# Yuki-11/CSBSR

Hardware: AMD Instinct MI355X
Metric: training imgs/s (448->1792 x4, PSPNet) (higher is better)
Workload: dtype fp16 storage / fp32 accumulate (detector forward: split fp16 hi+lo); 1 GPU; CSBSR KBPN x4 + PSPNet, beta=0.3, joint phase (iter 40000), per-GPU batch 8, LR 448x448 -> HR 1792x1792, fwd+loss+bwd+Adam; batch resident in HBM (H2D outside `value`, timed beside it as with_h2d_inside_step); full-size synthetic crack images degraded on the device; global_batch=8, micro_batch=8, parallelism=dp1

## Files before the change

csbsr_amd/csrc/conv_common.h:

```cpp
#pragma once
#include "common.h"

struct ConvK {
  csbsr_seg_t in[2];
  int N, H, W, OH, OW;
  int transposed, KHt, KWt;
  int stride, pad, dil;
  int ctot, c0;
  int Kp;
  int rows_p;
  const half_t* wt;
  int cout, coutp;
  half_t* out16; long o_sn, o_sy, o_sx;
  float* out32; long o32_sn, o32_sy, o32_sx, o32_sc;
  const float* bias;
  const float* cbias;
  int cb_mode;
  int act; float act_slope; const float* prelu;
  int res_mode; const half_t* res; long r_sn, r_sy, r_sx;
  const half_t* res2; long r2_sn, r2_sy, r2_sx;
  int accumulate;
  int stat_mode; float* stat;
  float out_scale;
  unsigned tiles_m, tiles_n;
// ... 284 lines not shown
      }
    }
    return;
  }
  if constexpr (BNSTAT) return;
  constexpr int NBATCH = 4 * (4 / NB);
  h8 rr[2][NB], oo[2][NB], mm[2][NB];
  auto load_batch = [&](int b, int st) __attribute__((always_inline)) {
    const int mp = b / (4 / NB), nb = (b % (4 / NB)) * NB;
    const int co = co0 + 16 * mp;
    const int coc = co < p.coutp ? co : p.coutp - 8;
#pragma unroll
    for (int r = 0; r < NB; ++r) {
      const int oyr = oyc[nb + r];
      rr[st][r] = h8{0, 0, 0, 0, 0, 0, 0, 0}; oo[st][r] = h8{0, 0, 0, 0, 0, 0, 0, 0}; mm[st][r] = h8{1, 1, 1, 1, 1, 1, 1, 1};
      if (fe.has_res) rr[st][r] = *reinterpret_cast<const h8*>(p.res + n * p.r_sn + oyr * p.r_sy + oxc * p.r_sx + coc);
      if (fe.has_old) oo[st][r] = *reinterpret_cast<const h8*>(p.out16 + n * p.o_sn + oyr * p.o_sy + oxc * p.o_sx + coc);
      if (fe.has_mask) mm[st][r] = *reinterpret_cast<const h8*>(p.mask + n * p.m_sn + oyr * p.m_sy + oxc * p.m_sx + coc);
    }
  };
  load_batch(0, 0);
#pragma unroll
  for (int b = 0; b < NBATCH; ++b) {
    if (b + 1 < NBATCH) load_batch(b + 1, (b + 1) & 1);
    const int mp = b / (4 / NB), nb = (b % (4 / NB)) * NB;
    const int co = co0 + 16 * mp;
    const int coc = co < p.coutp ? co : p.coutp - 8;
#pragma unroll
    for (int r = 0; r < NB; ++r) {
      float v[8], t[8];
#pragma unroll
      for (int e = 0; e < 8; ++e) v[e] = acc[mp >> 1][nb + r][8 * (mp & 1) + e];
      conv_epilogue_fast_values<true, BNSTAT>(fe, v, bias[mp], co, rr[b & 1][r], oo[b & 1][r], bsum[mp], bsq[mp], mm[b & 1][r], t, valid[nb + r] && co < p.coutp);
      split_store_rs(rs, (rowoff[nb + r] + pixoff + 2 * coc) | (co >= p.coutp ? (int)0x80000000 : 0), fe.o_lo, t);
        __builtin_amdgcn_sched_barrier(0);
    }
  }
}
#endif

template <int CPR, int NW>
__device__ __forceinline__ void conv_epilogue_flush_stats(const ConvK& p, float* sStat, int BN, int local_col, int co, float (&ssum)[8], float (&ssq)[8]) {
  if (p.stat_mode == CSBSR_STAT_NONE) return;
  const bool sq = p.stat_mode == CSBSR_STAT_BN;
#pragma unroll
  for (int e = 0; e < 8; ++e) {
    float a = co < p.coutp ? ssum[e] : 0.f, b = (sq && co < p.coutp) ? ssq[e] : 0.f;
#pragma unroll
    for (int o = CPR; o < 64; o <<= 1) { a += __shfl_xor(a, o, 64); if (sq) b += __shfl_xor(b, o, 64); }
    ssum[e] = a; ssq[e] = b;
  }
  const int wid = threadIdx.x >> 6;
  const bool mine = (threadIdx.x & 63) < CPR && co < p.coutp;
#pragma unroll 1
  for (int w = 0; w < NW; ++w) {
    if (wid == w && mine) {
#pragma unroll
      for (int e = 0; e < 8; ++e) {
        sStat[local_col + e] += ssum[e];
        if (sq) sStat[BN + local_col + e] += ssq[e];
      }
    }
    lds_barrier();
  }
}
__device__ __forceinline__ void conv_epilogue_store_stats(const ConvK& p, const float* sStat, int BN, int cout0, size_t row) {
  const int tid = threadIdx.x;
  if (p.stat_mode == CSBSR_STAT_NONE || tid >= BN || cout0 + tid >= p.coutp) return;
  float* r = p.stat_part + row * p.stat_ld + cout0 + tid;
  r[0] = sStat[tid];
  if (p.stat_mode == CSBSR_STAT_BN) r[p.coutp] = sStat[BN + tid];
}
struct ConvStatPlan { long rows; int tps; };
static inline int conv_stat_prepare(ConvK& p, int BM, int nphase, ConvStatPlan& pl, hipStream_t st) {
  pl.rows = 0; pl.tps = 0;
  p.stat_part = nullptr; p.stat_ld = 0; p.hw_pad = 0;
  if (p.stat_mode == CSBSR_STAT_NONE) return 0;
  if (p.stat_mode == CSBSR_STAT_SAMPLE_SUM) {
    CSBSR_CHECK(!p.transposed, "conv: per-sample sums of a transposed convolution are not built");
    if (p.tile2d) pl.tps = (p.OW / 16) * (p.OH / (BM / 16));
    else {
      p.hw_pad = round_up(p.OH * p.OW, BM);
      pl.tps = p.hw_pad / BM;
      p.tiles_m = (unsigned)(p.N * pl.tps);
    }
  }
  pl.rows = (long)p.tiles_m * nphase;
  p.stat_ld = (p.stat_mode == CSBSR_STAT_BN ? 2 : 1) * (long)p.coutp;
  p.stat_part = csbsr_red_scratch(pl.rows * p.stat_ld);
  CSBSR_NEED_SCRATCH(p.stat_part, "conv (fused statistics)");
  if (p.transposed && hipMemsetAsync(p.stat_part, 0, (size_t)pl.rows * p.stat_ld * 4, st) != hipSuccess) {
    csbsr_set_error("conv: memset of the statistics rows failed");
    return 2;
  }
  return 0;
}
static inline int conv_stat_finish(const ConvK& p, const ConvStatPlan& pl, hipStream_t st) {
  if (p.stat_mode == CSBSR_STAT_BN) return csbsr_sum_partials(p.stat_part, (int)pl.rows, p.stat_ld, 2 * p.coutp, p.stat, st);
  if (p.stat_mode == CSBSR_STAT_SAMPLE_SUM) return csbsr_sum_partials_batched(p.stat_part, pl.tps, p.stat_ld, p.coutp, p.stat, p.N, p.coutp, st);
  return 0;
}

__device__ __forceinline__ void conv_epilogue_direct_tile(const ConvK& p, const f16v& acc, int cbase ,
                                                          float slope, int n, int oy, int ox, const float* bias_tab = nullptr,
                                                          const EpiFast* fe = nullptr) {
  if (n < 0) return;
  const int hi = (threadIdx.x & 63) >> 5;
#pragma unroll
  for (int pair = 0; pair < 2; ++pair) {
    float v[8];
#pragma unroll
    for (int j = 0; j < 4; ++j) {
      const unsigned a = __float_as_uint(acc[8 * pair + j]), b = __float_as_uint(acc[8 * pair + 4 + j]);
      auto r = __builtin_amdgcn_permlane32_swap(a, b, false, false);
      v[j] = __uint_as_float(r[0]);
      v[4 + j] = __uint_as_float(r[1]);
    }
    const int co = cbase + 16 * pair + 8 * hi;
    if (co >= p.coutp) continue;
    float bias[8];
#pragma unroll
    for (int e = 0; e < 8; ++e) bias[e] = bias_tab ? bias_tab[co + e] : ((p.bias && co + e < p.cout) ? p.bias[co + e] : 0.f);
    float s0[8], s1[8];
    if (fe && fe->ok && !fe->bn) {
      half_t* o = p.out16 + n * p.o_sn + oy * p.o_sy + ox * p.o_sx + co;
      h8 rr = {0, 0, 0, 0, 0, 0, 0, 0}, oo = {0, 0, 0, 0, 0, 0, 0, 0};
      if (fe->has_res) rr = *reinterpret_cast<const h8*>(p.res + n * p.r_sn + oy * p.r_sy + ox * p.r_sx + co);
      if (fe->has_old) oo = *reinterpret_cast<const h8*>(o);
      float brow[8];
      if (fe->has_cb) conv_class_bias_row(p, bias, co, n, oy, ox, brow);
      else {
#pragma unroll
        for (int e = 0; e < 8; ++e) brow[e] = bias[e];
      }
      if (fe->has_res || fe->has_old) conv_epilogue_fast_row<true, false>(*fe, v, brow, co, o, rr, oo, s0, s1);
      else conv_epilogue_fast_row<false, false>(*fe, v, brow, co, o, rr, oo, s0, s1);
      continue;
    }
    conv_epilogue_row(p, v, bias, slope, co, n, oy, ox, s0, s1);
  }
}

enum { CONVK_IGEMM32 = 0, CONVK_IGEMM64, CONVK_IGEMM128, CONVK_GLDS128, CONVK_GLDS256, CONVK_THIN_COUT, CONVK_THIN_CIN, CONVK_GLDS256W, CONVK_HR, CONVK_TP, CONVK_X3, CONVK_THIN_TP, CONVK_X3S, CONVK_THIN_CIN2, CONVK_GLDS64, CONVK_THIN_SC, CONVK_THIN_TPD, CONVK_X3F, CONVK_X3SF, CONVK_X3W, CONVK_X3N };
extern thread_local int g_last_conv_kernel;
int conv_desc_to_k(const csbsr_conv_desc_t* d, ConvK& k);
bool conv_thin_eligible(const ConvK& k);
int conv_thin_launch(const ConvK& k, hipStream_t st);
void conv_thin_enable(int on);
bool conv_thin_cin_eligible(const ConvK& k, int creal);
int conv_thin_cin_launch(const ConvK& k, int creal, hipStream_t st);
bool conv_thin_cin2_eligible(const ConvK& k, int creal);
int conv_thin_cin2_launch(const ConvK& k, int creal, hipStream_t st);
void conv_thin_cin2_enable(int on);
int conv_thin_cin2_dact_launch(const ConvK& k, const csbsr_conv_desc_t* d, hipStream_t st);
extern "C" int32_t csbsr_conv_thin_dact_eligible(const csbsr_conv_desc_t* d);
bool conv_thin_tp_eligible(const ConvK& k, int creal, bool second_seg);
int conv_thin_tp_launch(const ConvK& k, hipStream_t st);
bool conv_thin_sc_eligible(const ConvK& k);
int conv_thin_sc_launch(const ConvK& k, hipStream_t st);
void conv_thin_sc_enable(int on);
bool conv_thin_tpd_eligible(const ConvK& k, int KH);
int conv_thin_tpd_launch(const ConvK& k, int KH, hipStream_t st);
void conv_thin_tpd_enable(int on);
bool conv_glds_eligible(const ConvK& k);
int conv_glds_launch(const ConvK& k, int nphase, long maxM, hipStream_t st);
```

csbsr_amd/csrc/conv_igemm_glds.hip:

```cpp
#include "common.h"
#include "csbsr_debug.h"
#include "conv_common.h"
#include <type_traits>

#ifdef CSBSR_TS
__device__ unsigned long long g_ts[8 * 262144];
#define TS(i) do { if (threadIdx.x == 0 && blockIdx.x < 262144) g_ts[(size_t)blockIdx.x * 8 + (i)] = wall_clock64(); } while (0)
extern "C" int csbsr_debug_read_ts(void* dst, long n) { return (int)hipMemcpyFromSymbol(dst, HIP_SYMBOL(g_ts), n * 8); }
#else
#define TS(i)
#endif
template <int BM, int NWM, int NSTAGE, int CT = 1, bool FS = false, bool GK = false>
__global__ __launch_bounds__(NWM * 128) void conv_igemm_glds_kernel(const ConvK p, const half_t* __restrict__ zero_page) {
  constexpr int BN = CT ? 128 * CT : 64, BKG = 64;
  constexpr int TA = CT ? 2 * CT : 1;
  constexpr int SOW = BN > 128 ? 128 : BN;
  constexpr int NW = NWM * 2, NT = NW * 64;
  constexpr int XI = BM / 8, WI = BN / 8;
  constexpr int NI = (XI + WI) / NW;
  constexpr int NXI = XI / NW;
  constexpr int STAGE_BYTES = (BM + BN) * 128;
  constexpr int RING_BYTES = NSTAGE * STAGE_BYTES;
  constexpr int OUT_LD = 64 + 4;
  constexpr int EPI_BYTES = BM * SOW * 4;
// ... 330 lines not shown
#pragma unroll
  for (int a = 0; a < (TA < 2 ? TA : 2); ++a)
#pragma unroll
    for (int b = 0; b < 2; ++b) {
      const int pix = wm * 64 + b * 32 + (lane & 31);
#pragma unroll
      for (int q = 0; q < 4; ++q) {
        const int slot = (wn * (SOW / 2) + a * 32 + 8 * q + 4 * (lane >> 5)) >> 2;
        const f16v& t = acc[2 * hh + a][b];
        f4 v = {t[4 * q + 0], t[4 * q + 1], t[4 * q + 2], t[4 * q + 3]};
        *reinterpret_cast<f4*>(sO + pix * SOW + ((slot ^ (pix & 15)) << 2)) = v;
      }
    }
  lds_barrier();
  if (hh == 0) TS(5);
  const int lcol = CT != 2 ? cc8 * 8 : (cc8 >> 3) * 128 + hh * 64 + (cc8 & 7) * 8;
  const int co = cout0 + lcol;
  float bias[8], ssum[8], ssq[8];
#pragma unroll
  for (int e = 0; e < 8; ++e) { bias[e] = sBias[lcol + e]; ssum[e] = ssq[e] = 0.f; }
  if (fe.ok) {
    constexpr int RPT = BM / RSTEP, EG = CT == 2 ? 2 : (RPT < 8 ? RPT : 8);
    static_assert(RPT % EG == 0, "rows per thread must split into groups");
    auto rows = [&](auto EXTRA, auto BNSTAT) {
#pragma unroll 1
      for (int g = 0; g < RPT / EG; ++g) {
        h8 rr[EG], oo[EG], mm[EG];
        long ooff[EG];
        bool live[EG];
#pragma unroll
        for (int i = 0; i < EG; ++i) {
          const int grow = tid / CPR + (g * EG + i) * RSTEP;
          const int n = sRow[grow * 3];
          live[i] = n >= 0 && co < p.coutp;
          ooff[i] = sOOff[grow] + co;
          rr[i] = h8{0, 0, 0, 0, 0, 0, 0, 0}; oo[i] = h8{0, 0, 0, 0, 0, 0, 0, 0}; mm[i] = h8{1, 1, 1, 1, 1, 1, 1, 1};
          if constexpr (decltype(EXTRA)::value) {
            if (live[i]) {
              if (fe.has_res || fe.has_mask) {
                const int oyo = py + sRow[grow * 3 + 1] * o_step, oxo = px + sRow[grow * 3 + 2] * o_step;
                if (fe.has_res) rr[i] = *reinterpret_cast<const h8*>(p.res + n * p.r_sn + oyo * p.r_sy + oxo * p.r_sx + co);
                if (fe.has_mask) mm[i] = *reinterpret_cast<const h8*>(p.mask + n * p.m_sn + oyo * p.m_sy + oxo * p.m_sx + co);
              }
              if (fe.has_old) oo[i] = *reinterpret_cast<const h8*>(p.out16 + ooff[i]);
            }
          }
        }
#pragma unroll
        for (int i = 0; i < EG; ++i) {
          if (!live[i]) continue;
          const int row = tid / CPR + (g * EG + i) * RSTEP;
          const f4 v0 = *reinterpret_cast<const f4*>(sO + row * SOW + (((2 * cc8) ^ (row & 15)) << 2));
          const f4 v1 = *reinterpret_cast<const f4*>(sO + row * SOW + (((2 * cc8 + 1) ^ (row & 15)) << 2));
          const float v[8] = {v0[0], v0[1], v0[2], v0[3], v1[0], v1[1], v1[2], v1[3]};
          if (fe.has_cb) {
            float brow[8];
            conv_class_bias_row(p, bias, co, sRow[row * 3], py + sRow[row * 3 + 1] * o_step, px + sRow[row * 3 + 2] * o_step, brow);
            conv_epilogue_fast_row<decltype(EXTRA)::value, decltype(BNSTAT)::value>(fe, v, brow, co, p.out16 + ooff[i], rr[i], oo[i], ssum, ssq, mm[i]);
            continue;
          }
          conv_epilogue_fast_row<decltype(EXTRA)::value, decltype(BNSTAT)::value>(fe, v, bias, co, p.out16 + ooff[i], rr[i], oo[i], ssum, ssq, mm[i]);
        }
      }
    };
    const bool extra = fe.has_res || fe.has_old || fe.has_mask;
    if (fe.bn) { if (extra) rows(std::true_type{}, std::true_type{}); else rows(std::false_type{}, std::true_type{}); }
    else { if (extra) rows(std::true_type{}, std::false_type{}); else rows(std::false_type{}, std::false_type{}); }
    if (fe.bn) conv_epilogue_flush_stats<CPR, NW>(p, sStat, BN, lcol, co, ssum, ssq);
  } else {
    constexpr int RPT = BM / RSTEP, EG = 2;
#pragma unroll 1
    for (int g = 0; g < RPT / EG; ++g) {
      EpiPre pre[EG];
      int rn[EG], roy[EG], rox[EG];
#pragma unroll
      for (int i = 0; i < EG; ++i) {
        const int grow = tid / CPR + (g * EG + i) * RSTEP;
        const int n = sRow[grow * 3];
        rn[i] = (n < 0 || co >= p.coutp) ? -1 : n;
        roy[i] = py + sRow[grow * 3 + 1] * o_step;
        rox[i] = px + sRow[grow * 3 + 2] * o_step;
        if (rn[i] >= 0) conv_epilogue_prefetch(p, co, rn[i], roy[i], rox[i], pre[i]);
      }
#pragma unroll
      for (int i = 0; i < EG; ++i) {
        if (rn[i] < 0) continue;
        const int row = tid / CPR + (g * EG + i) * RSTEP;
        float v[8];
        const f4 v0 = *reinterpret_cast<const f4*>(sO + row * SOW + (((2 * cc8) ^ (row & 15)) << 2));
        const f4 v1 = *reinterpret_cast<const f4*>(sO + row * SOW + (((2 * cc8 + 1) ^ (row & 15)) << 2));
        v[0] = v0[0]; v[1] = v0[1]; v[2] = v0[2]; v[3] = v0[3]; v[4] = v1[0]; v[5] = v1[1]; v[6] = v1[2]; v[7] = v1[3];
        conv_epilogue_row(p, v, bias, slope, co, rn[i], roy[i], rox[i], ssum, ssq, &pre[i]);
      }
    }
    conv_epilogue_flush_stats<CPR, NW>(p, sStat, BN, lcol, co, ssum, ssq);
  }
  };
  epi_pass(std::integral_constant<int, 0>{});
  if constexpr (CT == 2) epi_pass(std::integral_constant<int, 1>{});
  TS(6);
  conv_epilogue_store_stats(p, sStat, BN, cout0, (size_t)zph * p.tiles_m + tile_m);
}

static half_t* g_zero_page = nullptr;
static int g_glds_phase_flat = 1;
static int g_glds_tile2d = 1;
static int g_glds_tap_group = 1;
static int g_glds_wide = 1;
static int g_glds_narrow = 1;
static int g_glds_gk = 1;

template <int BM, int NWM, int NSTAGE, int CT = 1, bool FS = false, bool GK = false>
static int launch_glds(const ConvK& k, int nphase, long maxM, hipStream_t st) {
  ConvK p = k;
  constexpr int BN = CT ? 128 * CT : 64, SOW = BN > 128 ? 128 : BN;
  p.tiles_m = (unsigned)((maxM + BM - 1) / BM);
  p.tile2d = (g_glds_tile2d && !k.transposed && k.KHt * k.KWt > 1 && k.OW % 16 == 0 && k.OH % (BM / 16) == 0) ? 1 : 0;
  p.tap_group = (!GK && g_glds_tap_group && !k.transposed && k.stride > 1 && k.dil == 1 && k.KHt > k.stride && k.KHt % k.stride == 0 &&
                 k.KWt > k.stride && k.KWt % k.stride == 0) ? 1 : 0;
  p.tiles_n = (unsigned)((k.coutp + BN - 1) / BN);
  constexpr int RING = NSTAGE * (BM + BN) * 128;
  constexpr int EPI = BM * SOW * 4;
  constexpr int SM_BYTES = (RING > EPI ? RING : EPI) + BM * (4 * 8 + 3 * 4) + 3 * BN * 4 + (GK ? 64 * 8 : 0);
  static_assert(SM_BYTES <= 160 * 1024, "LDS budget");
  static LdsAttrOnce attr;
  if (int e = csbsr_lds_attr(attr, reinterpret_cast<const void*>(conv_igemm_glds_kernel<BM, NWM, NSTAGE, CT, FS, GK>), SM_BYTES, "conv(glds)")) return e;
  if (!g_zero_page) {
    if (hipMalloc(reinterpret_cast<void**>(&g_zero_page), 256) != hipSuccess) { csbsr_set_error("conv(glds): zero page alloc failed"); return 2; }
    (void)hipMemset(g_zero_page, 0, 256);
  }
  p.nphase_flat = (g_glds_phase_flat && nphase > 1) ? nphase : 0;
  ConvStatPlan sp;
  if (int e = conv_stat_prepare(p, BM, nphase, sp, st)) return e;
  dim3 grid(p.tiles_m * p.tiles_n * (p.nphase_flat ? nphase : 1), 1, p.nphase_flat ? 1 : nphase);
  hipLaunchKernelGGL((conv_igemm_glds_kernel<BM, NWM, NSTAGE, CT, FS, GK>), grid, dim3(NWM * 128), SM_BYTES, st, p, g_zero_page);
  if (int e = conv_stat_finish(p, sp, st)) return e;
  CSBSR_LAUNCH_CHECK("csbsr_conv_forward(glds)");
  return 0;
}

static int g_glds_mode = 2;
extern "C" void csbsr_debug_set_conv_glds(int mode) {
  g_glds_mode = mode & 7;
  g_glds_phase_flat = (mode & 32) ? 0 : 1;
  g_glds_tap_group = (mode & 128) ? 0 : 1;
  g_glds_tile2d = (mode & 64) ? 0 : 1;
  g_glds_wide = (mode & 256) ? 0 : 1;
  g_glds_narrow = (mode & 1024) ? 0 : 1;
  g_glds_gk = (mode & 2048) ? 0 : 1;
  conv_thin_enable((mode & 16) ? 0 : 1);
  conv_thin_sc_enable((mode & 4096) ? 0 : 1);
  conv_thin_tpd_enable((mode & 8192) ? 0 : 1);
  conv_thin_cin2_enable((mode & 512) ? 0 : 1);
}

static bool conv_glds_general_k(const ConvK& k) { return k.fs ? (k.ctot / 2) % 32 != 0 : k.ctot % 64 != 0; }

bool conv_glds_eligible(const ConvK& k) {
  if (g_glds_mode == 0) return false;
  if (k.coutp <= 32 || (k.coutp <= 64 && !g_glds_narrow)) return false;
  if (conv_glds_general_k(k)) {
    if (!g_glds_gk || k.c0 != k.ctot || (k.fs ? k.ctot / 2 : k.ctot) < 32) return false;
  } else if (k.c0 != k.ctot && k.c0 % 64 != 0) return false;
  if (k.rows_p % (k.coutp <= 64 ? 64 : 128) != 0) return false;
  if (k.KHt * k.KWt > 64) return false;
  return true;
}

int conv_glds_launch(const ConvK& k, int nphase, long maxM, hipStream_t st) {
  const bool big = (g_glds_mode == 2 && !k.transposed && k.Kp >= 2304 && maxM >= 256 * 256) ||
                   (g_glds_mode == 2 && !k.transposed && k.Kp >= 512 && k.coutp >= 384 && maxM >= (1l << 22)) ||
                   (g_glds_mode == 3 && maxM >= 256 * 256);
  const int pad128 = (k.coutp + 127) / 128 * 128, pad256 = (k.coutp + 255) / 256 * 256;
  const bool wide = big && g_glds_wide && k.coutp >= 256 && pad256 * 8 <= pad128 * 9 + 64;
  const bool gk = conv_glds_general_k(k);
  const int tile = k.coutp <= 64 ? 0 : (!big ? 1 : (wide ? 3 : 2));
  g_last_conv_kernel = (tile == 0 ? CONVK_GLDS64 : (tile == 1 ? CONVK_GLDS128 : (tile == 3 ? CONVK_GLDS256W : CONVK_GLDS256))) |
                       ((k.fs ? 1 : 0) | (gk ? 2 : 0)) << 8;
#define GLDS_DISPATCH(FS_, GK_)                                                                      \
  switch (tile) {                                                                                    \
    case 0: return launch_glds<128, 2, 2, 0, FS_, GK_>(k, nphase, maxM, st);                        \
    case 1: return launch_glds<128, 2, 2, 1, FS_, GK_>(k, nphase, maxM, st);                        \
    case 3: return launch_glds<256, 4, 2, 2, FS_, GK_>(k, nphase, maxM, st);                        \
    default: return launch_glds<256, 4, 3, 1, FS_, GK_>(k, nphase, maxM, st);                       \
  }
  if (k.fs) { if (gk) { GLDS_DISPATCH(true, true) } else { GLDS_DISPATCH(true, false) } }
  if (gk) { GLDS_DISPATCH(false, true) }
  GLDS_DISPATCH(false, false)
#undef GLDS_DISPATCH
}
```

csbsr_amd/csrc/conv_thin.hip:

```cpp
#include "conv_common.h"

#define TN_TH 8
#define TN_TW 32
#define TN_HW (TN_TW + 2)
#define TN_HP ((TN_TH + 2) * TN_HW)
#define TN_MB ((TN_HP + 31) / 32)
#define TN_YLD 33

#define TN_TPW 1

__global__ __launch_bounds__(256) void conv_thin_cout_kernel(const ConvK p, int tiles_x, int tiles_y, int wld) {
  extern __shared__ __attribute__((aligned(16))) char smem[];
  half_t* sW = reinterpret_cast<half_t*>(smem);
  float* sY = reinterpret_cast<float*>(smem + (size_t)32 * wld * sizeof(half_t));
  const int tid = threadIdx.x, lane = tid & 63, wid = tid >> 6;
  int b = blockIdx.x;
  const int tx = b % tiles_x; b /= tiles_x;
  const int tyg = (tiles_y + TN_TPW - 1) / TN_TPW;
  const int ty0 = (b % tyg) * TN_TPW;
  const int n = b / tyg;
  const int CR = p.cout, ntap_rows = 9 * CR;

  {
    const int chunks_per_row = wld / 8;
// ... 250 lines not shown
  }
  const float aslope = p.act == CSBSR_ACT_RELU ? 0.f : (p.act == CSBSR_ACT_LRELU ? p.act_slope : 1.f);
  const float mslope = DACT ? *x.slope : 1.f, rsign = p.res_mode == CSBSR_RES_SUB ? -1.f : 1.f;
  float dpr = 0.f;
  const half_t* in0 = reinterpret_cast<const half_t*>(p.in[0].ptr);
  const unsigned per_img = (unsigned)(tiles_x * tiles_y), total = per_img * (unsigned)p.N;
  auto halo_load = [&](unsigned t) {
    h8 v = {0, 0, 0, 0, 0, 0, 0, 0};
    if (tid < TN_HP && t < total) {
      const int n = t / per_img;
      const unsigned r = t - n * per_img;
      const int hy = tid / TN_HW, hx = tid - hy * TN_HW;
      const int iy = (int)(r / tiles_x) * TN_TH + hy - 1, ix = (int)(r % tiles_x) * TN_TW + hx - 1;
      if ((unsigned)iy < (unsigned)p.H && (unsigned)ix < (unsigned)p.W)
        v = *reinterpret_cast<const h8*>(in0 + (long)n * p.in[0].sn + (long)iy * p.in[0].sy + (long)ix * p.in[0].sx);
    }
    return v;
  };
  unsigned t = blockIdx.x;
  if (t >= total) return;
  {
    const h8 v = halo_load(t);
    if (tid < TN_HP) *reinterpret_cast<h8*>(sIn + tid * 8) = v;
  }
  __syncthreads();
  int buf = 0;
  for (; t < total; t += gridDim.x) {
    const h8 hnext = halo_load(t + gridDim.x);
    const int n = t / per_img;
    const unsigned r_ = t - n * per_img;
    const int oy = (int)(r_ / tiles_x) * TN_TH + wid, ox = (int)(r_ % tiles_x) * TN_TW + pix;
    const bool live = oy < p.OH && ox < p.OW;
    const half_t* sI = sIn + buf * (TN_HP * 8);
    h8 pf[2];
#pragma unroll
    for (int s = 0; s < 2; ++s)
#pragma unroll
      for (int e = 0; e < 8; ++e) {
        const int k = 16 * s + 8 * hi + e;
        const int tap = k / CI, c = k - tap * CI;
        const int ky = tap / 3, kx = tap - ky * 3;
        pf[s][e] = tap < 9 ? sI[((wid + ky) * TN_HW + pix + kx) * 8 + c] : (half_t)0;
      }
    half_t* o = p.out16 + (live ? n * p.o_sn + oy * p.o_sy + ox * p.o_sx : 0) + 8 * hi;
    h8 ring[RD][2];
    h8 ringm[DACT ? RD : 1][2], ringr[DACT ? RD : 1][2];
    const half_t* mo = DACT ? p.mask + (live ? n * p.m_sn + oy * p.m_sy + ox * p.m_sx : 0) + 8 * hi : nullptr;
    const half_t* ro = DACT ? p.res + (live ? n * p.r_sn + oy * p.r_sy + ox * p.r_sx : 0) + 8 * hi : nullptr;
    half_t* dro = DACT ? x.dres + (live ? n * x.d_sn + oy * x.d_sy + ox * x.d_sx : 0) + 8 * hi : nullptr;
    auto piece_ok = [&](int ct, int pair) { return 32 * ct + 16 * pair + 8 * hi < p.coutp; };
    if (has_old) {
#pragma unroll
      for (int j = 0; j < RD; ++j)
#pragma unroll
        for (int pair = 0; pair < 2; ++pair) {
          const int off = piece_ok(j, pair) ? 32 * j + 16 * pair : 0;
          ring[j][pair] = *reinterpret_cast<const h8*>(o + off);
          if constexpr (DACT) { ringm[j][pair] = *reinterpret_cast<const h8*>(mo + off); ringr[j][pair] = *reinterpret_cast<const h8*>(ro + off); }
        }
    }
    for (int c4 = 0; c4 < nct; c4 += RD) {
#pragma unroll
      for (int j = 0; j < RD; ++j) {
        const int ct = c4 + j;
        const int ctc = ct < nct ? ct : nct - 1;
        const half_t* wrow = sWt + (size_t)(ctc * 32 + pix) * TK_WLD + 8 * hi;
        const h8 w0 = *reinterpret_cast<const h8*>(wrow);
        const h8 w1 = *reinterpret_cast<const h8*>(wrow + 16);
        f16v acc;
#pragma unroll
        for (int r = 0; r < 16; ++r) acc[r] = 0.f;
        acc = __builtin_amdgcn_mfma_f32_32x32x16_f16(w0, pf[0], acc, 0, 0, 0);
        acc = __builtin_amdgcn_mfma_f32_32x32x16_f16(w1, pf[1], acc, 0, 0, 0);
#pragma unroll
        for (int pair = 0; pair < 2; ++pair) {
          float v[8];
#pragma unroll
          for (int q = 0; q < 4; ++q) {
            const unsigned a = __float_as_uint(acc[8 * pair + q]), b = __float_as_uint(acc[8 * pair + 4 + q]);
            auto r = __builtin_amdgcn_permlane32_swap(a, b, false, false);
            v[q] = __uint_as_float(r[0]);
            v[4 + q] = __uint_as_float(r[1]);
          }
          const h8 old = ring[j][pair];
          h8 mk = {0, 0, 0, 0, 0, 0, 0, 0}, rs = {0, 0, 0, 0, 0, 0, 0, 0};
          if constexpr (DACT) { mk = ringm[j][pair]; rs = ringr[j][pair]; }
          if (has_old) {
            const int ctn = ct + RD;
            const int off = (ctn < nct && piece_ok(ctn, pair)) ? 32 * ctn + 16 * pair : 0;
            ring[j][pair] = *reinterpret_cast<const h8*>(o + off);
            if constexpr (DACT) { ringm[j][pair] = *reinterpret_cast<const h8*>(mo + off); ringr[j][pair] = *reinterpret_cast<const h8*>(ro + off); }
          }
          h8 hv, hd;
          const bool st_ok = live && ct < nct && piece_ok(ct, pair);
#pragma unroll
          for (int e = 0; e < 8; ++e) {
            float tv = v[e] * p.out_scale;
            tv = fmaxf(tv, tv * aslope);
            if (has_old) tv += (float)old[e];
            if constexpr (DACT) {
              const float y = (float)mk[e] - rsign * (float)rs[e];
              const bool pos = y > 0.f;
              hd[e] = (half_t)(rsign * tv);
              if (st_ok && !pos) dpr += tv * y;
              tv = pos ? tv : tv * mslope;
            }
            hv[e] = (half_t)tv;
          }
          if (st_ok) {
            *reinterpret_cast<h8*>(o + 32 * ct + 16 * pair) = hv;
            if constexpr (DACT) *reinterpret_cast<h8*>(dro + 32 * ct + 16 * pair) = hd;
          }
        }
      }
    }
    if (tid < TN_HP) *reinterpret_cast<h8*>(sIn + (buf ^ 1) * (TN_HP * 8) + tid * 8) = hnext;
    __syncthreads();
    buf ^= 1;
  }
  if constexpr (DACT) {
    __shared__ float sdp[8];
    for (int o_ = 1; o_ < 64; o_ <<= 1) dpr += __shfl_xor(dpr, o_, 64);
    if (lane == 0) sdp[wid] = dpr;
    __syncthreads();
    if (tid == 0) {
      float a = 0.f;
      for (int w_ = 0; w_ < 8; ++w_) a += sdp[w_];
      x.part[blockIdx.x] = a / mslope;
    }
  }
}

static int g_conv_thin2 = 1;
void conv_thin_cin2_enable(int on) { g_conv_thin2 = on; }

bool conv_thin_cin2_eligible(const ConvK& k, int creal) {
  if (!g_conv_thin2 || !conv_thin_cin_eligible(k, creal)) return false;
  if (k.bias || k.cbias || k.res_mode != CSBSR_RES_NONE || k.mask || k.out32 || !k.out16 || k.o_lo) return false;
  if (k.act != CSBSR_ACT_NONE && k.act != CSBSR_ACT_RELU && k.act != CSBSR_ACT_LRELU) return false;
  if (k.coutp % 8 != 0 || k.o_sx < k.coutp) return false;
  return true;
}

extern "C" int32_t csbsr_conv_thin_dact_eligible(const csbsr_conv_desc_t* d) {
  if (!d || !g_conv_thin2 || d->transposed || !d->mask || !d->mask_prelu || !d->dres || !d->res || d->dact_bias) return 0;
  if (d->res_mode != CSBSR_RES_ADD && d->res_mode != CSBSR_RES_SUB) return 0;
  if (!d->accumulate || d->act != CSBSR_ACT_NONE || d->bias || d->cbias || d->out32 || !d->out16 || d->o_lo || d->r_lo || d->stat_mode != CSBSR_STAT_NONE) return 0;
  if (d->KH != 3 || d->KW != 3 || d->stride != 1 || d->dil != 1 || d->pad != 1 || d->OH != d->H || d->OW != d->W) return 0;
  if (d->in[1].c != 0 || d->in[0].c != 8 || d->in[0].creal < 1 || d->in[0].creal > 3 || d->in[0].sx == 0) return 0;
  if (d->cout < 32 || d->cout > 1024 || d->coutp % 8 != 0 || d->o_sx < d->coutp || d->dr_sx < d->coutp) return 0;
  return 1;
}

int conv_thin_cin2_launch(const ConvK& k, int creal, hipStream_t st) {
  const int tiles_x = (k.OW + TN_TW - 1) / TN_TW, tiles_y = (k.OH + TN_TH - 1) / TN_TH;
  const int nct = (k.cout + 31) / 32;
  const size_t smem = ((size_t)nct * 32 * TK_WLD + (size_t)2 * TN_HP * 8) * sizeof(half_t);
  static size_t configured = 0;
  if (smem > configured) {
    if (hipFuncSetAttribute(reinterpret_cast<const void*>(conv_thin_cin2_kernel<false>), hipFuncAttributeMaxDynamicSharedMemorySize, (int)smem) != hipSuccess) {
      csbsr_set_error("conv(thin-in, streaming): cannot reserve %zu bytes of LDS", smem);
      return 1;
    }
    configured = smem;
  }
  const long total = (long)k.N * tiles_x * tiles_y;
  const unsigned g = (unsigned)(total < 512 ? total : 512);
  hipLaunchKernelGGL(conv_thin_cin2_kernel<false>, dim3(g), dim3(512), smem, st, k, tiles_x, tiles_y, creal, k.accumulate ? 1 : 0, Cin2Dact{});
  CSBSR_LAUNCH_CHECK("csbsr_conv_forward(thin-in, streaming)");
  return 0;
}

int conv_thin_cin2_dact_launch(const ConvK& k, const csbsr_conv_desc_t* d, hipStream_t st) {
  const int tiles_x = (k.OW + TN_TW - 1) / TN_TW, tiles_y = (k.OH + TN_TH - 1) / TN_TH;
  const int nct = (k.cout + 31) / 32;
  const size_t smem = ((size_t)nct * 32 * TK_WLD + (size_t)2 * TN_HP * 8) * sizeof(half_t);
  static size_t configured = 0;
  if (smem > configured) {
    if (hipFuncSetAttribute(reinterpret_cast<const void*>(conv_thin_cin2_kernel<true>), hipFuncAttributeMaxDynamicSharedMemorySize, (int)smem) != hipSuccess) {
      csbsr_set_error("conv(thin-in, streaming, dact): cannot reserve %zu bytes of LDS", smem);
      return 1;
    }
    configured = smem;
  }
  const long total = (long)k.N * tiles_x * tiles_y;
  const unsigned g = (unsigned)(total < 256 ? total : 256);
  Cin2Dact x;
  x.dres = reinterpret_cast<half_t*>(d->dres); x.d_sn = d->dr_sn; x.d_sy = d->dr_sy; x.d_sx = d->dr_sx;
  x.slope = d->mask_prelu;
  x.part = csbsr_red_scratch((long)g);
  CSBSR_NEED_SCRATCH(x.part, "conv(thin-in, dact)");
  hipLaunchKernelGGL(conv_thin_cin2_kernel<true>, dim3(g), dim3(512), smem, st, k, tiles_x, tiles_y, d->in[0].creal, 1, x);
  if (d->dact_prelu) { if (int e = csbsr_sum_partials(x.part, (int)g, 1, 1, d->dact_prelu, st)) return e; }
  CSBSR_LAUNCH_CHECK("csbsr_conv_forward(thin-in, streaming, dact)");
  return 0;
}

#define TP_ROW_MAX 1024
template <int CI>
__global__ __launch_bounds__(256) void conv_thin_tp_kernel(const ConvK p, int groups_per_phase) {
  const int tid = threadIdx.x;
  const int c8 = p.coutp >> 3;
  const int oct = tid % c8, pl = tid / c8;
  const int npl = 256 / c8;
  if (pl >= npl) return;
  const int s = p.stride;
  int b = blockIdx.x;
  const int rg = b % groups_per_phase; b /= groups_per_phase;
  const int py = b % s;
  const int n = b / s;
  const int px = pl % s, sub = pl / s, nsub = npl / s;
  const int by = (py + p.pad) / s, bx = (px + p.pad) / s;
  const int ph = py * s + px;
  const int co = oct * 8;
  static_assert(CI == 3, "channel pairs (c0, c1), (c2, pad)");
  h2 w2[4][2][8];
#pragma unroll
  for (int t = 0; t < 4; ++t)
#pragma unroll
    for (int e = 0; e < 8; ++e) {
      const half_t* wp = p.wt + ((size_t)ph * p.rows_p + co + e) * p.Kp + t * p.ctot;
      w2[t][0][e] = h2{wp[0], wp[1]};
      w2[t][1][e] = h2{wp[2], (half_t)0};
    }
  float bias[8];
#pragma unroll
  for (int e = 0; e < 8; ++e) bias[e] = (p.bias && co + e < p.cout) ? p.bias[co + e] : 0.f;
  const float slope = p.act == CSBSR_ACT_PRELU ? *p.prelu : (p.act == CSBSR_ACT_RELU ? 0.f : (p.act == CSBSR_ACT_NONE ? 1.f : p.act_slope));
  const float rsign = p.res_mode == CSBSR_RES_ADD ? 1.f : (p.res_mode == CSBSR_RES_SUB ? -1.f : 0.f);
  const half_t* in0 = reinterpret_cast<const half_t*>(p.in[0].ptr) + (long)n * p.in[0].sn;
  const int rows_per_group = (p.OH / s + groups_per_phase - 1) / groups_per_phase;
  __shared__ h8 srow[2][TP_ROW_MAX + 2];
  for (int r = 0; r < rows_per_group; ++r) {
    const int qy = rg * rows_per_group + r;
    const int oy = qy * s + py;
    if (oy >= p.OH) break;
    __syncthreads();
    for (int i = tid; i < 2 * (p.W + 2); i += 256) {
      const int tr = i / (p.W + 2), ix = i - tr * (p.W + 2) - 1, iy = qy + by - tr;
      h8 v = h8{0, 0, 0, 0, 0, 0, 0, 0};
      if ((unsigned)iy < (unsigned)p.H && (unsigned)ix < (unsigned)p.W) v = *reinterpret_cast<const h8*>(in0 + (long)iy * p.in[0].sy + (long)ix * p.in[0].sx);
      srow[tr][ix + 1] = v;
    }
    __syncthreads();
    for (int qx0 = sub; qx0 * s + px < p.OW; qx0 += 8 * nsub) {
      h8 rr[8];
#pragma unroll
      for (int u = 0; u < 8; ++u) {
        const int ox = (qx0 + u * nsub) * s + px;
        rr[u] = h8{0, 0, 0, 0, 0, 0, 0, 0};
        if (ox < p.OW && rsign != 0.f) rr[u] = *reinterpret_cast<const h8*>(p.res + n * p.r_sn + (long)oy * p.r_sy + (long)ox * p.r_sx + co);
      }
#pragma unroll
      for (int half = 0; half < 2; ++half) {
        h8 xv[4][4];
#pragma unroll
        for (int u = 0; u < 4; ++u) {
          const int qx = qx0 + (4 * half + u) * nsub, ox = qx * s + px;
          const bool live = ox < p.OW;
#pragma unroll
          for (int t = 0; t < 4; ++t) {
            const int ix = qx + bx - (t & 1);
            xv[u][t] = srow[t >> 1][live ? ix + 1 : 0];
          }
        }
#pragma unroll
        for (int u = 0; u < 4; ++u) {
          const int qx = qx0 + (4 * half + u) * nsub, ox = qx * s + px;
          if (ox >= p.OW) break;
          float acc[8];
#pragma unroll
          for (int e = 0; e < 8; ++e) acc[e] = 0.f;
#pragma unroll
          for (int t = 0; t < 4; ++t) {
            const h2 x01 = h2{xv[u][t][0], xv[u][t][1]}, x23 = h2{xv[u][t][2], (half_t)0};
#pragma unroll
            for (int e = 0; e < 8; ++e) {
              acc[e] = __builtin_amdgcn_fdot2(x01, w2[t][0][e], acc[e], false);
              acc[e] = __builtin_amdgcn_fdot2(x23, w2[t][1][e], acc[e], false);
            }
          }
          h8 hv;
#pragma unroll
          for (int e = 0; e < 8; ++e) {
            float t_ = acc[e] * p.out_scale + bias[e];
            t_ = t_ > 0.f ? t_ : t_ * slope;
            if (co + e >= p.cout) t_ = 0.f;
            t_ += rsign * (float)rr[4 * half + u][e];
            hv[e] = (half_t)t_;
          }
          *reinterpret_cast<h8*>(p.out16 + n * p.o_sn + (long)oy * p.o_sy + (long)ox * p.o_sx + co) = hv;
        }
      }
    }
  }
}

bool conv_thin_tp_eligible(const ConvK& k, int creal, bool second_seg) {
  if (!g_conv_thin || !k.transposed || second_seg) return false;
  if (k.KHt != 2 || k.KWt != 2 || k.stride < 2 || k.dil != 1 || k.pad >= k.stride) return false;
  if (k.ctot != 8 || creal != 3 || k.in[0].sx == 0 || k.W > TP_ROW_MAX) return false;
  if (k.OH != k.H * k.stride || k.OW != k.W * k.stride) return false;
  if (k.coutp < 8 || k.coutp > 128 || (256 / (k.coutp / 8)) % k.stride != 0 || 256 % (k.coutp / 8) != 0) return false;
  if (!k.out16 || k.out32 || k.o_lo || k.r_lo || k.cbias || k.mask || k.accumulate || k.stat_mode != CSBSR_STAT_NONE) return false;
  if (k.act == CSBSR_ACT_SIGMOID || (k.res_mode != CSBSR_RES_NONE && k.res_mode != CSBSR_RES_ADD && k.res_mode != CSBSR_RES_SUB)) return false;
  return true;
}

int conv_thin_tp_launch(const ConvK& k, hipStream_t st) {
// ... 226 lines not shown
```

csbsr_amd/utils/kernel_names.py:

```python
import re

_CONV = {0: "conv_igemm_kernel<32,4,1>", 1: "conv_igemm_kernel<64,2,2>", 2: "conv_igemm_kernel<128,2,2>", 5: "conv_thin_cout_kernel",
         6: "conv_thin_cin_kernel", 11: "conv_thin_tp_kernel", 13: "conv_thin_cin2_kernel", 15: "conv_thin_sc_kernel", 16: "conv_thin_tpd_kernel",
         10: "conv_x3_kernel<3>", 12: "conv_x3_kernel<2>", 17: "conv_x3_kernel<3,1024>", 18: "conv_x3_kernel<2,1024>"}
HEAD1_FWD, HEAD1_BWD_INPUT = 21, 22
_GLDS = {3: (128, 2, 2, 1), 4: (256, 4, 3, 1), 7: (256, 4, 2, 2), 14: (128, 2, 2, 0)}
_WGRAD = {0: "conv_wgrad_kernel<128,128,2,2>", 1: "conv_wgrad_kernel<128,256,2,4>", 2: "conv_wgrad_kernel<64,128,2,2>",
          3: "conv_wgrad_kernel<32,128,1,4>", 4: "conv_wgrad_thin_kernel", 5: "conv_wgrad_glds_kernel<128,128>",
          6: "conv_wgrad_glds_kernel<128,256>", 7: "conv_wgrad_glds_kernel<256,256>", 8: "conv_wgrad_hr_kernel",
          9: "conv_wgrad_glds_kernel<128,512>"}


def conv_row(kid):
    base, var = kid & 255, kid >> 8
    if base in _GLDS:
        bm, nwm, ns, ct = _GLDS[base]
        return f"conv_igemm_glds_kernel<{bm},{nwm},{ns},{ct},FS={var & 1},GK={(var >> 1) & 1}>"
    if base == 9:
        return f"conv_tp_kernel<res={var & 1},acc={(var >> 1) & 1},mask={(var >> 2) & 1},sums={(var >> 3) & 1}>"
    if base == 8:
        return (f"conv_hr_kernel<{7 if var & 1 else 4},stat={(var >> 4) & 1},taps={1 if var & 2 else 9},nct={2 if var & 4 else 1},"
                f"mask={(var >> 3) & 1},cb={(var >> 5) & 1}>")
    if base == 10 and var & 1:
        return "conv_x3_kernel<3,2048>"
    if base == 19:
        return f"conv_x3w_kernel<{var}>"
    if base in (HEAD1_FWD, HEAD1_BWD_INPUT):
        return "head1_fwd_kernel" if base == HEAD1_FWD else "head1_bwd_input_kernel"
    if base == 20:
        return "conv_x3n_kernel<%d,%d%s%s>" % (var & 1, (var >> 1) & 1, ",wide" if var & 4 else "", ",lean" if var & 8 else "")
    return _CONV.get(base, f"conv?{base}")


def wgrad_row(kid):
    return _WGRAD.get(kid, f"conv_wgrad?{kid}")


def family(row):
    return row.split("<", 1)[0]


def _b(x):
    return "1" if x in ("1", "true") else "0"


def canon(name):
    m = (re.search(r"conv_igemm_glds_kernelILi(\d+)ELi(\d+)ELi(\d+)ELi(\d+)ELb(\d)ELb(\d)E", name)
         or re.search(r"conv_igemm_glds_kernel<(\d+), (\d+), (\d+), (\d+), (\w+), (\w+)>", name))
    if m:
        g = m.groups()
        return "conv_igemm_glds_kernel<%s,%s,%s,%s,FS=%s,GK=%s>" % (g[0], g[1], g[2], g[3], _b(g[4]), _b(g[5]))
    m = re.search(r"conv_igemm_kernelILi(\d+)ELi(\d+)ELi(\d+)E", name) or re.search(r"conv_igemm_kernel<(\d+), (\d+), (\d+)>", name)
    if m:
        return "conv_igemm_kernel<%s,%s,%s>" % m.groups()
    m = re.search(r"conv_wgrad_glds_kernelILi(\d+)ELi(\d+)E", name) or re.search(r"conv_wgrad_glds_kernel<(\d+), (\d+)", name)
    if m:
        return "conv_wgrad_glds_kernel<%s,%s>" % m.groups()
    m = re.search(r"conv_wgrad_kernel<(\d+), (\d+), (\d+), (\d+)", name) or re.search(r"conv_wgrad_kernelILi(\d+)ELi(\d+)ELi(\d+)ELi(\d+)E", name)
    if m:
        return "conv_wgrad_kernel<%s,%s,%s,%s>" % m.groups()
    m = (re.search(r"conv_hr_kernelILi(\d+)ELb(\d)ELi(\d+)ELi(\d+)ELb(\d)ELb(\d)E", name)
         or re.search(r"conv_hr_kernel<(\d+), (\w+), (\d+), (\d+), (\w+), (\w+)>", name))
    if m:
        g = m.groups()
        return "conv_hr_kernel<%s,stat=%s,taps=%s,nct=%s,mask=%s,cb=%s>" % (g[0], _b(g[1]), g[2], g[3], _b(g[4]), _b(g[5]))
    m = re.search(r"conv_tp_kernelILi\d+ELb(\d)ELb(\d)ELb(\d)ELb(\d)E", name) or re.search(r"conv_tp_kernel<\d+, (\w+), (\w+), (\w+), (\w+)>", name)
    if m:
        return "conv_tp_kernel<res=%s,acc=%s,mask=%s,sums=%s>" % tuple(_b(x) for x in m.groups())
    m = (re.search(r"conv_x3n_kernelILb(\d)ELb(\d)ELb(\d)ELb(\d)E", name)
         or re.search(r"conv_x3n_kernel<(\w+), (\w+), (\w+), (\w+)>", name))
    if m:
        return "conv_x3n_kernel<%s,%s%s%s>" % (_b(m.group(1)), _b(m.group(2)), ",wide" if _b(m.group(3)) == "1" else "",
                                               ",lean" if _b(m.group(4)) == "1" else "")
    m = re.search(r"conv_x3w_kernelILi(\d)E", name) or re.search(r"conv_x3w_kernel<(\d)>", name)
    if m:
        return "conv_x3w_kernel<%s>" % m.group(1)
    m = re.search(r"conv_x3_kernelILi(\d)ELi(\d+)E", name) or re.search(r"conv_x3_kernel<(\d), (\d+)>", name)
    if m:
        return "conv_x3_kernel<%s>" % m.group(1) if m.group(2) == "0" else "conv_x3_kernel<%s,%s>" % m.groups()
    for k in ("conv_wgrad_hr_kernel", "conv_wgrad_thin_kernel", "conv_wgrad_kernel", "conv_thin_cout_kernel", "conv_thin_cin2_kernel", "conv_thin_cin_kernel",
              "conv_thin_tpd_kernel", "conv_thin_tp_kernel", "conv_thin_sc_kernel", "thin_tp_bwd_kernel", "epilogue_bwd_kernel", "unpack_wgrad_kernel",
              "head1_fwd_kernel", "head1_bwd_input_kernel", "bn_bwd_apply_kernel", "bn_bwd_reduce_kernel", "bn_apply_kernel", "channel_mean_sub_kernel", "round_weights_kernel"):
        if k in name:
            return k
    return name[:60]
```

Baseline: 8.316 imgs/s.

## Add persistent streaming thin-Cin conv kernel for 3-channel narrow-Cout layers

Adds a persistent-grid variant of the thin-input conv (Cin=3, Cout<=64) that loops over tiles with a double-buffered halo prefetch in LDS. It packs the 27 taps×channels into two MFMA K-slices and stages outputs per wave through LDS so each output row is written as coalesced 16-byte stores. The aim is to hide global load latency and improve write coalescing for the HR-resolution first conv layers. In exchange it uses more LDS and caps the grid at 512 blocks, which may limit occupancy on a large GPU.

```diff
diff --git a/csbsr_amd/csrc/conv_common.h b/csbsr_amd/csrc/conv_common.h
--- a/csbsr_amd/csrc/conv_common.h
+++ b/csbsr_amd/csrc/conv_common.h
@@ -460,6 +460,7 @@
 bool conv_thin_cin2_eligible(const ConvK& k, int creal);
 int conv_thin_cin2_launch(const ConvK& k, int creal, hipStream_t st);
 void conv_thin_cin2_enable(int on);
+void conv_thin_cin2n_enable(int on);
 int conv_thin_cin2_dact_launch(const ConvK& k, const csbsr_conv_desc_t* d, hipStream_t st);
 extern "C" int32_t csbsr_conv_thin_dact_eligible(const csbsr_conv_desc_t* d);
 bool conv_thin_tp_eligible(const ConvK& k, int creal, bool second_seg);
diff --git a/csbsr_amd/csrc/conv_igemm_glds.hip b/csbsr_amd/csrc/conv_igemm_glds.hip
--- a/csbsr_amd/csrc/conv_igemm_glds.hip
+++ b/csbsr_amd/csrc/conv_igemm_glds.hip
@@ -506,6 +506,7 @@
   conv_thin_sc_enable((mode & 4096) ? 0 : 1);
   conv_thin_tpd_enable((mode & 8192) ? 0 : 1);
   conv_thin_cin2_enable((mode & 512) ? 0 : 1);
+  conv_thin_cin2n_enable((mode & 16384) ? 0 : 1);
 }
 
 static bool conv_glds_general_k(const ConvK& k) { return k.fs ? (k.ctot / 2) % 32 != 0 : k.ctot % 64 != 0; }
diff --git a/csbsr_amd/csrc/conv_thin.hip b/csbsr_amd/csrc/conv_thin.hip
--- a/csbsr_amd/csrc/conv_thin.hip
+++ b/csbsr_amd/csrc/conv_thin.hip
@@ -426,9 +426,176 @@
   return 1;
 }
 
+#define TC2N_IN_LD (TN_HP * 8 + 8)
+#define TC2N_ST_LD (32 * 9 * 8)
+template <int NCT, bool OLD>
+__global__ __launch_bounds__(512, 2) void conv_thin_cin2n_kernel(const ConvK p, int tiles_x, int tiles_y) {
+  extern __shared__ __attribute__((aligned(16))) char smem[];
+  constexpr int CI = 3;
+  half_t* sWt = reinterpret_cast<half_t*>(smem);
+  half_t* sIn = sWt + NCT * 32 * TK_WLD;
+  half_t* sSt = sIn + 2 * TC2N_IN_LD;
+  const int tid = threadIdx.x, lane = tid & 63, hi = lane >> 5, pix = lane & 31;
+  const int wid = __builtin_amdgcn_readfirstlane(tid >> 6);
+  for (int id = tid; id < NCT * 32 * (TK_WLD / 8); id += 512) {
+    const h8 z = {0, 0, 0, 0, 0, 0, 0, 0};
+    *reinterpret_cast<h8*>(sWt + id * 8) = z;
+  }
+  if (tid < 16) sIn[(tid >> 3) * TC2N_IN_LD + TN_HP * 8 + (tid & 7)] = (half_t)0;
+  __syncthreads();
+  for (int id = tid; id < NCT * 32 * 9; id += 512) {
+    const int co = id / 9, tap = id - co * 9;
+    const h8 v = *reinterpret_cast<const h8*>(p.wt + (size_t)co * p.Kp + tap * 8);
+    for (int c = 0; c < CI; ++c) sWt[co * TK_WLD + tap * CI + c] = v[c];
+  }
+  const float aslope = p.act == CSBSR_ACT_RELU ? 0.f : (p.act == CSBSR_ACT_LRELU ? p.act_slope : 1.f);
+  int goff[2][8];
+#pragma unroll
+  for (int s = 0; s < 2; ++s)
+#pragma unroll
+    for (int e = 0; e < 8; ++e) {
+      const int k = 16 * s + 8 * hi + e;
+      const int tap = k / CI, c = k - tap * CI;
+      const int ky = tap / 3, kx = tap - ky * 3;
+      goff[s][e] = tap < 9 ? ((wid + ky) * TN_HW + pix + kx) * 8 + c : TN_HP * 8;
+    }
+  const int cp8 = p.coutp >> 3, pitch = cp8 | 1;
+  half_t* stg = sSt + wid * TC2N_ST_LD;
+  half_t* stw = stg + pix * pitch * 8 + 8 * hi;
+  int roff[4];
+#pragma unroll
+  for (int i = 0; i < 4; ++i) {
+    const int j = lane + 64 * i, px_ = j / cp8;
+    roff[i] = j < 32 * cp8 ? (px_ * pitch + (j - px_ * cp8)) * 8 : -1;
+  }
+  const bool dense = p.o_sx == p.coutp;
+  const half_t* in0 = reinterpret_cast<const half_t*>(p.in[0].ptr);
+  const unsigned per_img = (unsigned)(tiles_x * tiles_y), total = per_img * (unsigned)p.N;
+  auto halo_load = [&](unsigned t) {
+    h8 v = {0, 0, 0, 0, 0, 0, 0, 0};
+    if (tid < TN_HP && t < total) {
+      const int n = t / per_img;
+      const unsigned r = t - n * per_img;
+      const int hy = tid / TN_HW, hx = tid - hy * TN_HW;
+      const int iy = (int)(r / tiles_x) * TN_TH + hy - 1, ix = (int)(r % tiles_x) * TN_TW + hx - 1;
+      if ((unsigned)iy < (unsigned)p.H && (unsigned)ix < (unsigned)p.W)
+        v = *reinterpret_cast<const h8*>(in0 + (long)n * p.in[0].sn + (long)iy * p.in[0].sy + (long)ix * p.in[0].sx);
+    }
+    return v;
+  };
+  unsigned t = blockIdx.x;
+  if (t >= total) return;
+  {
+    const h8 v = halo_load(t);
+    if (tid < TN_HP) *reinterpret_cast<h8*>(sIn + tid * 8) = v;
+  }
+  __syncthreads();
+  int buf = 0;
+  for (; t < total; t += gridDim.x) {
+    const h8 hnext = halo_load(t + gridDim.x);
+    const int n = t / per_img;
+    const unsigned r_ = t - n * per_img;
+    const int ox0 = (int)(r_ % tiles_x) * TN_TW;
+    const int oy = (int)(r_ / tiles_x) * TN_TH + wid, ox = ox0 + pix;
+    const bool live = oy < p.OH && ox < p.OW;
+    const half_t* sI = sIn + buf * TC2N_IN_LD;
+    h8 pf[2];
+#pragma unroll
+    for (int s = 0; s < 2; ++s)
+#pragma unroll
+      for (int e = 0; e < 8; ++e) pf[s][e] = sI[goff[s][e]];
+    half_t* o = p.out16 + (live ? n * p.o_sn + oy * p.o_sy + ox * p.o_sx : 0) + 8 * hi;
+    half_t* orow = p.out16 + n * p.o_sn + (oy < p.OH ? oy : 0) * p.o_sy + ox0 * p.o_sx;
+    const bool staged = dense && oy < p.OH && ox0 + TN_TW <= p.OW && (reinterpret_cast<size_t>(orow) & 127) == 0;
+    auto piece_ok = [&](int ct, int pair) { return 32 * ct + 16 * pair + 8 * hi < p.coutp; };
+    h8 ring[NCT][2];
+    if constexpr (OLD) {
+#pragma unroll
+      for (int ct = 0; ct < NCT; ++ct)
+#pragma unroll
+        for (int pair = 0; pair < 2; ++pair) ring[ct][pair] = *reinterpret_cast<const h8*>(o + (piece_ok(ct, pair) ? 32 * ct + 16 * pair : 0));
+    }
+    h8 hv[NCT][2];
+#pragma unroll
+    for (int ct = 0; ct < NCT; ++ct) {
+      const half_t* wrow = sWt + (size_t)(ct * 32 + pix) * TK_WLD + 8 * hi;
+      const h8 w0 = *reinterpret_cast<const h8*>(wrow);
+      const h8 w1 = *reinterpret_cast<const h8*>(wrow + 16);
+      f16v acc;
+#pragma unroll
+      for (int r = 0; r < 16; ++r) acc[r] = 0.f;
+      acc = __builtin_amdgcn_mfma_f32_32x32x16_f16(w0, pf[0], acc, 0, 0, 0);
+      acc = __builtin_amdgcn_mfma_f32_32x32x16_f16(w1, pf[1], acc, 0, 0, 0);
+#pragma unroll
+      for (int pair = 0; pair < 2; ++pair) {
+        float v[8];
+#pragma unroll
+        for (int q = 0; q < 4; ++q) {
+          const unsigned a = __float_as_uint(acc[8 * pair + q]), b = __float_as_uint(acc[8 * pair + 4 + q]);
+          auto r = __builtin_amdgcn_permlane32_swap(a, b, false, false);
+          v[q] = __uint_as_float(r[0]);
+          v[4 + q] = __uint_as_float(r[1]);
+        }
+#pragma unroll
+        for (int e = 0; e < 8; ++e) {
+          float tv = v[e] * p.out_scale;
+          tv = fmaxf(tv, tv * aslope);
+          if constexpr (OLD) tv += (float)ring[ct][pair][e];
+          hv[ct][pair][e] = (half_t)tv;
+        }
+      }
+    }
+    if (staged) {
+#pragma unroll
+      for (int ct = 0; ct < NCT; ++ct)
+#pragma unroll
+        for (int pair = 0; pair < 2; ++pair)
+          if (ct + 1 < NCT || piece_ok(ct, pair)) *reinterpret_cast<h8*>(stw + 32 * ct + 16 * pair) = hv[ct][pair];
+      __builtin_amdgcn_fence(__ATOMIC_RELEASE, "wavefront");
+      __builtin_amdgcn_wave_barrier();
+      __builtin_amdgcn_fence(__ATOMIC_ACQUIRE, "wavefront");
+      h8 ln[4];
+#pragma unroll
+      for (int i = 0; i < 4; ++i) ln[i] = *reinterpret_cast<const h8*>(stg + (roff[i] >= 0 ? roff[i] : 0));
+#pragma unroll
+      for (int i = 0; i < 4; ++i)
+        if (roff[i] >= 0) *reinterpret_cast<h8*>(orow + (lane + 64 * i) * 8) = ln[i];
+    } else if (live) {
+#pragma unroll
+      for (int ct = 0; ct < NCT; ++ct)
+#pragma unroll
+        for (int pair = 0; pair < 2; ++pair)
+          if (ct + 1 < NCT || piece_ok(ct, pair)) *reinterpret_cast<h8*>(o + 32 * ct + 16 * pair) = hv[ct][pair];
+    }
+    if (tid < TN_HP) *reinterpret_cast<h8*>(sIn + (buf ^ 1) * TC2N_IN_LD + tid * 8) = hnext;
+    __syncthreads();
+    buf ^= 1;
+  }
+}
+
+static int g_conv_thin2n = 1;
+void conv_thin_cin2n_enable(int on) { g_conv_thin2n = on; }
+
+template <int NCT, bool OLD>
+static int conv_thin_cin2n_launch(const ConvK& k, int tiles_x, int tiles_y, unsigned g, hipStream_t st) {
+  const size_t smem = ((size_t)NCT * 32 * TK_WLD + (size_t)2 * TC2N_IN_LD + (size_t)8 * TC2N_ST_LD) * sizeof(half_t);
+  static LdsAttrOnce once;
+  if (int e = csbsr_lds_attr(once, reinterpret_cast<const void*>(conv_thin_cin2n_kernel<NCT, OLD>), (int)smem, "conv(thin-in, streaming, narrow)")) return e;
+  hipLaunchKernelGGL((conv_thin_cin2n_kernel<NCT, OLD>), dim3(g), dim3(512), smem, st, k, tiles_x, tiles_y);
+  CSBSR_LAUNCH_CHECK("csbsr_conv_forward(thin-in, streaming, narrow)");
+  return 0;
+}
+
 int conv_thin_cin2_launch(const ConvK& k, int creal, hipStream_t st) {
   const int tiles_x = (k.OW + TN_TW - 1) / TN_TW, tiles_y = (k.OH + TN_TH - 1) / TN_TH;
   const int nct = (k.cout + 31) / 32;
+  if (g_conv_thin2n && k.cout <= 64 && creal == 3) {
+    const long total = (long)k.N * tiles_x * tiles_y;
+    const unsigned g = (unsigned)(total < 512 ? total : 512);
+    g_last_conv_kernel = CONVK_THIN_CIN2 | 1 << 8;
+    if (nct == 1) return k.accumulate ? conv_thin_cin2n_launch<1, true>(k, tiles_x, tiles_y, g, st) : conv_thin_cin2n_launch<1, false>(k, tiles_x, tiles_y, g, st);
+    return k.accumulate ? conv_thin_cin2n_launch<2, true>(k, tiles_x, tiles_y, g, st) : conv_thin_cin2n_launch<2, false>(k, tiles_x, tiles_y, g, st);
+  }
   const size_t smem = ((size_t)nct * 32 * TK_WLD + (size_t)2 * TN_HP * 8) * sizeof(half_t);
   static size_t configured = 0;
   if (smem > configured) {
diff --git a/csbsr_amd/utils/kernel_names.py b/csbsr_amd/utils/kernel_names.py
--- a/csbsr_amd/utils/kernel_names.py
+++ b/csbsr_amd/utils/kernel_names.py
@@ -23,6 +23,8 @@
                 f"mask={(var >> 3) & 1},cb={(var >> 5) & 1}>")
     if base == 10 and var & 1:
         return "conv_x3_kernel<3,2048>"
+    if base == 13 and var & 1:
+        return "conv_thin_cin2n_kernel"
     if base == 19:
         return f"conv_x3w_kernel<{var}>"
     if base in (HEAD1_FWD, HEAD1_BWD_INPUT):
@@ -78,7 +80,7 @@
     m = re.search(r"conv_x3_kernelILi(\d)ELi(\d+)E", name) or re.search(r"conv_x3_kernel<(\d), (\d+)>", name)
     if m:
         return "conv_x3_kernel<%s>" % m.group(1) if m.group(2) == "0" else "conv_x3_kernel<%s,%s>" % m.groups()
-    for k in ("conv_wgrad_hr_kernel", "conv_wgrad_thin_kernel", "conv_wgrad_kernel", "conv_thin_cout_kernel", "conv_thin_cin2_kernel", "conv_thin_cin_kernel",
+    for k in ("conv_wgrad_hr_kernel", "conv_wgrad_thin_kernel", "conv_wgrad_kernel", "conv_thin_cout_kernel", "conv_thin_cin2n_kernel", "conv_thin_cin2_kernel", "conv_thin_cin_kernel",
               "conv_thin_tpd_kernel", "conv_thin_tp_kernel", "conv_thin_sc_kernel", "thin_tp_bwd_kernel", "epilogue_bwd_kernel", "unpack_wgrad_kernel",
               "head1_fwd_kernel", "head1_bwd_input_kernel", "bn_bwd_apply_kernel", "bn_bwd_reduce_kernel", "bn_apply_kernel", "channel_mean_sub_kernel", "round_weights_kernel"):
         if k in name:
```

Measured after the change: 8.293 imgs/s. About the same (-0.3%).
